# laoreja/HPLFlowNet

Hardware: AMD Instinct MI355X
Metric: point-pairs/sec + EPE3D, N=8192 FlyingThings3D, 1/2/4/8 MI355X (higher is better)
Workload: dtype f32 (wide layers: fp32 operands as scaled fp16 pairs, 3 partial products, fp32 accumulate); 1 GPU; full HPLFlowNet inference (7 levels, 19.3M params, random init), FT3D-like synthetic pair, N=8192, bs=1 per GPU; num_points=8192, step_includes_lattice_build=True, forward_streams=3, lattices_under_construction=3, exact_fallback_launches=0, lattice_launches_per_pair=34

## Files before the change

hplflownet_amd/csrc/gconv3.hip:

```cpp
#include "common.h"
#include "gconv_common.h"

#include <stdlib.h>
#include <string>
#include <type_traits>

using namespace hpl;
using namespace hpl_gc;

typedef __bf16 bf16x8 __attribute__((ext_vector_type(8)));
typedef __bf16 bf16x2 __attribute__((ext_vector_type(2)));
typedef _Float16 f16x8 __attribute__((ext_vector_type(8)));
typedef _Float16 f16x2 __attribute__((ext_vector_type(2)));
typedef float float2_t __attribute__((ext_vector_type(2)));
typedef unsigned u32x4 __attribute__((ext_vector_type(4)));
typedef unsigned u32x2 __attribute__((ext_vector_type(2)));


namespace {

__device__ __forceinline__ void split2(float x0, float x1, unsigned &h, unsigned &m, unsigned &l) {
    const float2_t v = {x0, x1};
    h = __builtin_bit_cast(unsigned, __builtin_convertvector(v, bf16x2));
    const float r0 = x0 - __builtin_bit_cast(float, h << 16), r1 = x1 - __builtin_bit_cast(float, h & 0xffff0000u);
    const float2_t rv = {r0, r1};
    m = __builtin_bit_cast(unsigned, __builtin_convertvector(rv, bf16x2));
    const float s0 = r0 - __builtin_bit_cast(float, m << 16), s1 = r1 - __builtin_bit_cast(float, m & 0xffff0000u);
    const float2_t sv = {s0, s1};
    l = __builtin_bit_cast(unsigned, __builtin_convertvector(sv, bf16x2));
}

__device__ __forceinline__ void split2h(float x0, float x1, float s, unsigned &h, unsigned &l) {
    const float2_t v = {x0 * s, x1 * s};
    const f16x2 hh = __builtin_convertvector(v, f16x2);
    h = __builtin_bit_cast(unsigned, hh);
    const float2_t hf = __builtin_convertvector(hh, float2_t);
    const float2_t r = {v.x - hf.x, v.y - hf.y};
    l = __builtin_bit_cast(unsigned, __builtin_convertvector(r, f16x2));
}

__device__ __forceinline__ void split2h_resid(float x0, float x1, float s, unsigned &h, unsigned &l) {
    const float2_t v = {x0 * s, x1 * s};
    const f16x2 hh = __builtin_convertvector(v, f16x2);
    const float2_t hf = __builtin_convertvector(hh, float2_t);
    const float2_t r = {v.x - hf.x, v.y - hf.y};
    const f16x2 ll = __builtin_convertvector(r, f16x2);
    const float2_t lf = __builtin_convertvector(ll, float2_t);
    constexpr float K = (float)(1 << RESID_SHIFT);
    const float2_t r2 = {(r.x - lf.x) * K, (r.y - lf.y) * K};
    const f16x2 h2 = __builtin_convertvector(r2, f16x2);
    h = __builtin_bit_cast(unsigned, h2);
    const float2_t h2f = __builtin_convertvector(h2, float2_t);
    const float2_t q = {r2.x - h2f.x, r2.y - h2f.y};
    l = __builtin_bit_cast(unsigned, __builtin_convertvector(q, f16x2));
}

constexpr int BM3 = 128;

template <int WGN, int F_LDS, int NB, int PL, bool GUARD = false>
__device__ __forceinline__ void gconv3_body(const GParams &p, const unsigned block) {
    static_assert(PL == 2 || PL == 3, "operand planes: 2 (fp16 pairs) or 3 (bf16 triples)");
    static_assert(!GUARD || PL == 2, "the range guard belongs to the fp16-pair form");
    bool tripped = false;
    if constexpr (PL == 2) tripped = guard_tripped(p.a_amax, p.a_guard);
    if constexpr (GUARD) { if (!tripped) return; }
    constexpr int BM = BM3, BN = 64 * WGN, NT = 128 * WGN;
    constexpr int ROWS_PP = NT / 4;
    constexpr int A_PASSES = 2 * BM / ROWS_PP;
    constexpr int HALF_PASSES = A_PASSES / 2;
    constexpr int A_STAGE = PL * 2 * BM * 16;
    constexpr int B_STAGE = PL * 2 * BN * 16;
    constexpr int NA = 3;
    static_assert(NB == 3 || NB == 4, "weight ring of 3 or 4 stages");
    constexpr int ASETS = NB - 1;
    constexpr int B_BASE = NA * A_STAGE;
    constexpr int B_CHUNKS_PER_WAVE = PL;
    constexpr int KLIST = 1024;
    constexpr bool PP = WGN == 4;
    static_assert(A_PASSES == 2 || A_PASSES == 4, "two halves of a slice per thread");
    __shared__ __attribute__((aligned(16))) unsigned char smem[NA * A_STAGE + NB * B_STAGE + ((F_LDS + 1) * BM + BM + 8) * 4 + KLIST * 2];
    int *Is = reinterpret_cast<int *>(smem + NA * A_STAGE + NB * B_STAGE);
    int *Vs = Is + (F_LDS + 1) * BM;
    int *tapmask_s = Vs + BM;
    unsigned short *Ks = reinterpret_cast<unsigned short *>(tapmask_s + 8);

    int tile_m, tile_n;
    tile_coords(p, tile_m, tile_n, block);
    if (tile_m < 0) return;
    const int64_t m0 = (int64_t)tile_m * BM;
    const int n0 = tile_n * BN;
    const int t = threadIdx.x, lane = t & 63;
    const int wave = __builtin_amdgcn_readfirstlane(t >> 6);
    const int wm = wave / WGN, wn = wave % WGN;
    const int li = lane & 31, hi = lane >> 5;

    const bool probe = p.clock_probe && (block & 63) == 0 && t == 0;
    long long probe_c = 0, probe_w = 0;
    if (probe) { probe_c = (long long)__builtin_readcyclecounter(); probe_w = (long long)__builtin_amdgcn_s_memrealtime(); }

    if (p.tile_idx && p.tile_bm == BM) {
        const int32_t *ti = p.tile_idx + (int64_t)tile_m * p.F * BM;
        if (t < 8) tapmask_s[t] = p.tile_mask[(int64_t)tile_m * 8 + t];
        for (int r = t; r < BM; r += NT) {
            const int64_t m = m0 + r;
            Vs[r] = (m < p.M) ? (p.row_perm ? p.row_perm[m] : (int)m) : -1;
        }
        for (int i = t; i < (F_LDS + 1) * BM; i += NT) {
            const int row = (i < p.F * BM) ? ti[i] : -1;
            Is[i] = row >= 0 ? row * (int)(p.lda * 4) : (int)0x80000000;
        }
    } else {
        if (t < 8) tapmask_s[t] = 0;
        for (int r = t; r < BM; r += NT) {
            const int64_t m = m0 + r;
            Vs[r] = (m < p.M) ? (p.row_perm ? p.row_perm[m] : (int)m) : -1;
        }
        __syncthreads();
        int mybits = 0;
        for (int i = t; i < F_LDS * BM; i += NT) {
            const int f = i / BM, r = i - f * BM;
            const int v = Vs[r];
            int row = -1;
            if (v >= 0 && f < p.F) row = p.nbr ? p.nbr[(int64_t)f * p.nbr_stride + v] : (int)((int64_t)f * p.reg_stride + v);
            Is[i] = row >= 0 ? row * (int)(p.lda * 4) : (int)0x80000000;
            mybits |= (row >= 0) ? (1 << f) : 0;
        }
        for (int i = F_LDS * BM + t; i < (F_LDS + 1) * BM; i += NT) Is[i] = (int)0x80000000;
        if (mybits) {
            atomicOr(tapmask_s, mybits);
            atomicOr(tapmask_s + 2 + ((t % BM) >> 5), mybits);
        }
    }
    __syncthreads();
    const int tapmask = __builtin_amdgcn_readfirstlane(tapmask_s[0]);
    const bool blockskip = p.C >= BK;
    int bmask[2];
#pragma unroll
    for (int i = 0; i < 2; ++i) bmask[i] = __builtin_amdgcn_readfirstlane(tapmask_s[2 + wm * 2 + i]);
    const int nk = (p.K + BK - 1) / BK;
    if (wave == 0) {
        int count = 0;
        for (int base = 0; base < nk; base += 64) {
            const int kt = base + lane;
            bool need = false;
            int f_lo = 0;
            if (kt < nk) {
                f_lo = (kt * BK) / p.C;
                const int f_hi = min((kt * BK + BK - 1) / p.C, p.F - 1);
                int bits = 0;
                for (int f = f_lo; f <= f_hi; ++f) bits |= 1 << f;
                need = (tapmask & bits) != 0;
            }
            const unsigned long long bal = __ballot(need);
            if (need) {
                int e = kt;
                e |= (f_lo << 10) | ((blockskip && (kt * BK + BK - 1) / p.C > f_lo && f_lo + 1 < p.F) ? (1 << 14) : 0);
                Ks[count + __popcll(bal & ((1ull << lane) - 1ull))] = (unsigned short)e;
            }
            count += __popcll(bal);
        }
        if (lane == 0) tapmask_s[1] = count;
    }
    __syncthreads();
    int nsl = __builtin_amdgcn_readfirstlane(tapmask_s[1]);
    int split = 0;
    if (p.splits > 1) {
        const int ngrid = p.row_perm && p.col_share > 0 ? p.tiles_n * p.col_share * p.col_rows : p.tiles_m * p.tiles_n;
        split = (int)block / ngrid;
        const int k_lo = (int)((int64_t)nk * split / p.splits), k_hi = (int)((int64_t)nk * (split + 1) / p.splits);
        auto below = [&](int kt) {
            int a = 0, b = nsl;
            while (a < b) {
                const int mid = (a + b) >> 1;
                if ((int)(Ks[mid] & 1023) < kt) a = mid + 1; else b = mid;
            }
            return a;
        };
        const int lo = below(k_lo), hi_e = below(k_hi);
        __syncthreads();
        if (lo > 0) {
            unsigned short mine[KLIST / (128 * WGN) + 1];
            int cnt = 0;
            for (int i = t; i < hi_e - lo; i += NT) mine[cnt++] = Ks[lo + i];
            __syncthreads();
            cnt = 0;
            for (int i = t; i < hi_e - lo; i += NT) Ks[i] = mine[cnt++];
        }
        __syncthreads();
        nsl = hi_e - lo;
    }

    constexpr unsigned OOB = 0x80000000u;
    const int32x4_t rsrc_a = make_rsrc(p.A, (int)p.a_bytes);
    const int k4 = t & 3, arow0 = t >> 2;
    const unsigned w3_bytes = (unsigned)(p.w_bytes / 2);
    __amdgpu_buffer_rsrc_t rsrc_b[PL];
#pragma unroll
    for (int pl = 0; pl < PL; ++pl)
        rsrc_b[pl] = __builtin_amdgcn_make_buffer_rsrc(
            const_cast<unsigned char *>(reinterpret_cast<const unsigned char *>(p.Wt3) + (int64_t)pl * p.w3_plane_stride),
            (short)0, (int)w3_bytes, 0x00020000);
    const unsigned ldw16 = (unsigned)p.ldw * 16u;

    float4_t ra[ASETS][A_PASSES];
    int a_rows[A_PASSES], a_c[A_PASSES];
    auto load_a_rows = [&](int e) {
        const int f0 = (e >> 10) & 15;
        const int c0 = (e & 1023) * BK - f0 * p.C;
#pragma unroll
        for (int i = 0; i < A_PASSES; ++i) {
            int c = c0 + ((i & 1) * 4 + k4) * 4, f = f0;
            const bool wrap = c >= p.C;
            c = wrap ? c - p.C : c;
            f += wrap ? 1 : 0;
            a_rows[i] = Is[f * BM + arow0 + (i >> 1) * ROWS_PP];
            a_c[i] = c;
        }
    };
    auto load_a_issue = [&](auto set_tag) {
        constexpr int SET = decltype(set_tag)::value;
        const int32x4_t rs = rsrc_a;
#pragma unroll
        for (int i = 0; i < A_PASSES; ++i) {
            float4_t &dst = ra[SET][i];
            const unsigned o = (unsigned)a_rows[i] + (unsigned)a_c[i] * 4u;
            asm volatile("buffer_load_dwordx4 %0, %1, %2, 0 offen" : "=v"(dst) : "v"(o), "s"(rs) : "memory");
        }
    };
    auto load_a = [&](auto set_tag, int e) {
        load_a_rows(e);
        load_a_issue(set_tag);
    };
    auto pin = [&](auto set_tag) {
        constexpr int SET = decltype(set_tag)::value;
#pragma unroll
        for (int i = 0; i < A_PASSES; ++i) {
            float4_t &x = ra[SET][i];
            asm volatile("" : "+v"(x));
        }
    };
    auto a_slot = [](int row, int kb) { return row ^ ((((row >> 5) & 3) << 1) ^ (kb << 2)); };
    const int kb_w = (t >> 1) & 1;
    float s_a = 1.f, s_out = 1.f, s_out2 = 1.f;
    if constexpr (PL == 2) {
        s_a = split_scale(p.a_amax[0]);
        s_out = split_unscale(s_a);
        if constexpr (GUARD) s_out *= 1.0f / (float)(1 << RESID_SHIFT);
        s_out2 = split_unscale(split_scale(p.w_amax[0]));
    }
    auto store_a = [&](auto set_tag, int h, int st, int j) {
        constexpr int SET = decltype(set_tag)::value;
        const float4_t v = h ? ra[SET][2 * j + 1] : ra[SET][2 * j];
        const int row = arow0 + j * ROWS_PP;
        unsigned char *base = smem + st * A_STAGE + (kb_w * BM + a_slot(row, kb_w)) * 16 + (t & 1) * 8;
        if constexpr (PL == 2) {
            unsigned h0, l0, h1, l1;
            if constexpr (GUARD) {
                split2h_resid(v.x, v.y, s_a, h0, l0);
                split2h_resid(v.z, v.w, s_a, h1, l1);
            } else {
                split2h(v.x, v.y, s_a, h0, l0);
                split2h(v.z, v.w, s_a, h1, l1);
            }
            *reinterpret_cast<u32x2 *>(base) = u32x2{h0, h1};
            *reinterpret_cast<u32x2 *>(base + 2 * BM * 16) = u32x2{l0, l1};
        } else {
            unsigned h0, m0_, l0, h1, m1, l1;
            split2(v.x, v.y, h0, m0_, l0);
            split2(v.z, v.w, h1, m1, l1);
            *reinterpret_cast<u32x2 *>(base) = u32x2{h0, h1};
            *reinterpret_cast<u32x2 *>(base + 2 * BM * 16) = u32x2{m0_, m1};
            *reinterpret_cast<u32x2 *>(base + 4 * BM * 16) = u32x2{l0, l1};
        }
    };
    const unsigned b_colofs = ((unsigned)(n0 + wn * 64 + lane) < (unsigned)p.ldw) ? (unsigned)(n0 + wn * 64 + lane) * 16u : OOB;
    auto load_b = [&](int kt, int h, int st) {
        const unsigned kbg = (unsigned)(kt * (BK / 8) + h * 2 + wm);
        const unsigned off = kbg * ldw16 + b_colofs;
#pragma unroll
        for (int pl = 0; pl < PL; ++pl)
            __builtin_amdgcn_raw_ptr_buffer_load_lds(
                rsrc_b[pl],
                (__attribute__((address_space(3))) void *)(smem + B_BASE + st * B_STAGE + ((pl * 2 + wm) * BN + wn * 64) * 16),
                16, (int)off, 0, 0, 0);
    };

    floatx16 acc[2][2];
#pragma unroll
    for (int i = 0; i < 2; ++i)
#pragma unroll
        for (int j = 0; j < 2; ++j)
#pragma unroll
            for (int r = 0; r < 16; ++r) acc[i][j][r] = 0.f;

    unsigned a_rofs[2];
#pragma unroll
    for (int i = 0; i < 2; ++i) {
        const int row = wm * 64 + i * 32 + li;
        a_rofs[i] = (unsigned)((hi * BM + (row ^ ((((row >> 5) & 3) << 1) ^ (hi << 2)))) * 16);
    }
    const unsigned b_rofs = (unsigned)(B_BASE + (hi * BN + wn * 64 + li) * 16);

    using S0 = std::integral_constant<int, 0>;
    using S1 = std::integral_constant<int, 1>;
    using T = std::true_type;
    using Fl = std::false_type;
    auto wait_vm_lgkm0 = [](auto n_tag) {
        constexpr int N = decltype(n_tag)::value;
        __builtin_amdgcn_s_waitcnt((N & 0xF) | ((N >> 4) << 14) | (0x7 << 4) | (0x0 << 8));
    };

    using S2 = std::integral_constant<int, 2>;
    if (nsl > 0) {
        int ks_cb = 0;
        int ks_reg = (int)Ks[min(lane, KLIST - 1)];
        auto ks_at = [&](int x) { return __builtin_amdgcn_readlane(ks_reg, x - ks_cb); };
        auto ks_advance = [&](int sl) {
            if (sl - ks_cb >= 32) { ks_cb += 32; ks_reg = (int)Ks[min(ks_cb + lane, KLIST - 1)]; }
        };
        auto kt_at = [&](int sl) { return ks_at(sl) & 1023; };
#pragma unroll
        for (int g = 0; g < NB - 1; ++g)
            if (g / 2 < nsl) load_b(kt_at(g / 2), g & 1, g);
        load_a(S0{}, ks_at(0));
        wait_vm_lgkm0(S0{});
        pin(S0{});
#pragma unroll
        for (int j = 0; j < HALF_PASSES; ++j) { store_a(S0{}, 0, 0, j); store_a(S0{}, 1, 1, j); }
        if (nsl > 1) load_a(S1{}, ks_at(1));
        if constexpr (ASETS == 3) { if (nsl > 2) load_a(S2{}, ks_at(2)); }
        wait_vm_lgkm0(S0{});
        asm volatile("s_barrier" ::: "memory");

        if (PP && wm == 1) asm volatile("s_barrier" ::: "memory");

        int sta = 0, stb = 0;
        auto halfstep = [&](int e_cur, int h, auto b_tag, int kt_b, int hb_b, auto w_tag, auto setw_tag, auto l_tag, auto setl_tag,
                            int kt_l, auto inflight_tag) {
            constexpr bool B = decltype(b_tag)::value, W = decltype(w_tag)::value, L = decltype(l_tag)::value;
            const int sta2 = sta >= 1 ? sta - 1 : 2;
            const int stb2 = stb >= 1 ? stb - 1 : NB - 1;
            const unsigned char *sa = smem + sta * A_STAGE;
            const unsigned char *sb = smem + stb * B_STAGE;
            bool need[2];
            {
                const int f_lo = (e_cur >> 10) & 15, two = (e_cur >> 14) & 1;
#pragma unroll
                for (int i = 0; i < 2; ++i)
                    need[i] = !blockskip || (((bmask[i] >> f_lo) | (two ? (bmask[i] >> (f_lo + 1)) : 0)) & 1);
            }
            u32x4 af[PL][2], bf[PL][2];
            constexpr int NQ = PL == 3 ? 6 : 3;
            constexpr int PA[6] = {0, 0, 1, 0, PL == 3 ? 2 : 0, 1};
            constexpr int PB[6] = {0, 1, 0, PL == 3 ? 2 : 0, 0, 1};
            auto mfma = [&](const u32x4 &a, const u32x4 &b, floatx16 &c) {
                if constexpr (PL == 3)
                    c = __builtin_amdgcn_mfma_f32_32x32x16_bf16(__builtin_bit_cast(bf16x8, b), __builtin_bit_cast(bf16x8, a), c, 0, 0, 0);
                else
                    c = __builtin_amdgcn_mfma_f32_32x32x16_f16(__builtin_bit_cast(f16x8, b), __builtin_bit_cast(f16x8, a), c, 0, 0, 0);
            };
            if constexpr (PP) {
#pragma unroll
                for (int pl = 0; pl < PL; ++pl)
#pragma unroll
                    for (int i = 0; i < 2; ++i) {
                        af[pl][i] = *reinterpret_cast<const u32x4 *>(sa + a_rofs[i] + pl * 2 * BM * 16);
                        bf[pl][i] = *reinterpret_cast<const u32x4 *>(sb + b_rofs + pl * 2 * BN * 16 + i * 32 * 16);
                    }
                wait_vm_lgkm0(inflight_tag);
                __builtin_amdgcn_sched_barrier(0);
                asm volatile("s_barrier" ::: "memory");
                __builtin_amdgcn_sched_barrier(0);
                auto others = [&]() {
                    if constexpr (B) load_b(kt_b, hb_b, stb2);
                    if constexpr (L) { load_a_issue(setl_tag); load_a_rows(kt_l); }
                    if constexpr (W) {
                        if (h == 0) pin(setw_tag);
#pragma unroll
                        for (int j = 0; j < HALF_PASSES; ++j) store_a(setw_tag, h, sta2, j);
                    }
                };
                if (need[0] || need[1]) {
#pragma unroll
                    for (int q = 0; q < NQ; ++q)
#pragma unroll
                        for (int i = 0; i < 2; ++i)
#pragma unroll
                            for (int j = 0; j < 2; ++j) mfma(af[PA[q]][i], bf[PB[q]][j], acc[i][j]);
                    others();
#pragma unroll
                    for (int k = 0; k < 4 * NQ; ++k) {
                        __builtin_amdgcn_sched_group_barrier(0x008, 1, 0);
                        __builtin_amdgcn_sched_group_barrier(0x006, 4, 0);
                        if (k % 3 == 0) __builtin_amdgcn_sched_group_barrier(0x020, 1, 0);
                        if (k % 4 == 1) __builtin_amdgcn_sched_group_barrier(0x100, 1, 0);
                        if (k % 4 == 3) __builtin_amdgcn_sched_group_barrier(0x200, 1, 0);
                    }
                } else {
                    others();
                }
                __builtin_amdgcn_sched_barrier(0);
                asm volatile("s_barrier" ::: "memory");
                __builtin_amdgcn_sched_barrier(0);
                sta = sta == 2 ? 0 : sta + 1;
                stb = stb == NB - 1 ? 0 : stb + 1;
                return;
            }
            if (need[0] || need[1]) {
#pragma unroll
                for (int pl = 0; pl < PL; ++pl)
#pragma unroll
                    for (int i = 0; i < 2; ++i) {
                        af[pl][i] = *reinterpret_cast<const u32x4 *>(sa + a_rofs[i] + pl * 2 * BM * 16);
                        bf[pl][i] = *reinterpret_cast<const u32x4 *>(sb + b_rofs + pl * 2 * BN * 16 + i * 32 * 16);
                    }
            }
            if constexpr (B) load_b(kt_b, hb_b, stb2);
            if constexpr (L) load_a_rows(kt_l);
            if constexpr (W) { if (h == 0) pin(setw_tag); }
            auto rest = [&]() {
                if constexpr (L) load_a_issue(setl_tag);
                if constexpr (W) {
#pragma unroll
                    for (int j = 0; j < HALF_PASSES; ++j) store_a(setw_tag, h, sta2, j);
                }
            };
            if (need[0] || need[1]) {
#pragma unroll
                for (int q = 0; q < NQ; ++q)
#pragma unroll
                    for (int i = 0; i < 2; ++i)
#pragma unroll
                        for (int j = 0; j < 2; ++j) mfma(af[PA[q]][i], bf[PB[q]][j], acc[i][j]);
                rest();
#pragma unroll
                for (int k = 0; k < 4 * NQ; ++k) {
                    __builtin_amdgcn_sched_group_barrier(0x008, 1, 0);
                    __builtin_amdgcn_sched_group_barrier(0x006, 4, 0);
                    if (k % 4 == 0) __builtin_amdgcn_sched_group_barrier(0x020, 1, 0);
                    if (k % 4 == 3) __builtin_amdgcn_sched_group_barrier(0x200, 1, 0);
                }
            } else {
                rest();
            }
            wait_vm_lgkm0(inflight_tag);
            asm volatile("s_barrier" ::: "memory");
            sta = sta == 2 ? 0 : sta + 1;
            stb = stb == NB - 1 ? 0 : stb + 1;
        };
        constexpr int NLB = B_CHUNKS_PER_WAVE, NLA = A_PASSES;
        auto slice_steady = [&](int sl, auto u_tag) {
            constexpr int U = decltype(u_tag)::value;
            using SW = std::integral_constant<int, (U + 1) % ASETS>;
            using SL = std::integral_constant<int, U % ASETS>;
            ks_advance(sl);
            const int e = ks_at(sl);
            const int k1 = kt_at(sl + 1), kl = ks_at(sl + ASETS);
            if constexpr (PP) {
                halfstep(e, 0, T{}, k1, 1, T{}, SW{}, T{}, SL{}, ks_at(sl + ASETS + 1), std::integral_constant<int, NLB>{});
                halfstep(e, 1, T{}, kt_at(sl + 2), 0, T{}, SW{}, Fl{}, SL{}, 0, std::integral_constant<int, NLB + NLA>{});
            } else
            if constexpr (NB == 3) {
                halfstep(e, 0, T{}, k1, 0, T{}, SW{}, T{}, SL{}, kl, std::integral_constant<int, NLB + NLA>{});
                halfstep(e, 1, T{}, k1, 1, T{}, SW{}, Fl{}, SL{}, 0, std::integral_constant<int, NLB>{});
            } else {
                halfstep(e, 0, T{}, k1, 1, T{}, SW{}, T{}, SL{}, kl, std::integral_constant<int, 2 * NLB + NLA>{});
                halfstep(e, 1, T{}, kt_at(sl + 2), 0, T{}, SW{}, Fl{}, SL{}, 0, std::integral_constant<int, 2 * NLB + NLA>{});
            }
        };
        auto slice_tail = [&](int sl, auto u_tag) {
            constexpr int U = decltype(u_tag)::value;
            using SW = std::integral_constant<int, (U + 1) % ASETS>;
            using SL = std::integral_constant<int, U % ASETS>;
            using Z = std::integral_constant<int, 0>;
            ks_advance(sl);
            const int e = ks_at(sl);
            const bool w = sl + 1 < nsl, l = sl + ASETS < nsl;
            const int kl = l ? ks_at(sl + ASETS + (PP ? 1 : 0)) : 0;
            {
                const int gb = 2 * sl + NB - 1;
                const bool b = gb / 2 < nsl;
                const int kb = b ? kt_at(gb / 2) : 0;
                if (b && w && l) halfstep(e, 0, T{}, kb, gb & 1, T{}, SW{}, T{}, SL{}, kl, Z{});
                else if (b && w) halfstep(e, 0, T{}, kb, gb & 1, T{}, SW{}, Fl{}, SL{}, 0, Z{});
                else if (w) halfstep(e, 0, Fl{}, 0, 0, T{}, SW{}, Fl{}, SL{}, 0, Z{});
                else if (b) halfstep(e, 0, T{}, kb, gb & 1, Fl{}, SW{}, Fl{}, SL{}, 0, Z{});
                else halfstep(e, 0, Fl{}, 0, 0, Fl{}, SW{}, Fl{}, SL{}, 0, Z{});
            }
            {
                const int gb = 2 * sl + 1 + NB - 1;
                const bool b = gb / 2 < nsl;
                const int kb = b ? kt_at(gb / 2) : 0;
                if (b && w) halfstep(e, 1, T{}, kb, gb & 1, T{}, SW{}, Fl{}, SL{}, 0, Z{});
                else if (w) halfstep(e, 1, Fl{}, 0, 0, T{}, SW{}, Fl{}, SL{}, 0, Z{});
                else if (b) halfstep(e, 1, T{}, kb, gb & 1, Fl{}, SW{}, Fl{}, SL{}, 0, Z{});
                else halfstep(e, 1, Fl{}, 0, 0, Fl{}, SW{}, Fl{}, SL{}, 0, Z{});
            }
        };
        if constexpr (PP) load_a_rows(ks_at(ASETS));
        int sl = 0;
        for (; sl + 2 * ASETS < nsl; sl += ASETS) {
            slice_steady(sl, S0{});
            slice_steady(sl + 1, S1{});
            if constexpr (ASETS == 3) slice_steady(sl + 2, S2{});
        }
        for (; sl < nsl; sl += ASETS) {
            slice_tail(sl, S0{});
            if (sl + 1 < nsl) slice_tail(sl + 1, S1{});
            if constexpr (ASETS == 3) { if (sl + 2 < nsl) slice_tail(sl + 2, S2{}); }
        }
        if (PP && wm == 0) asm volatile("s_barrier" ::: "memory");
    }
    if constexpr (PL == 2) {
#pragma unroll
        for (int i = 0; i < 2; ++i)
#pragma unroll
            for (int j = 0; j < 2; ++j)
#pragma unroll
                for (int r = 0; r < 16; ++r) acc[i][j][r] = acc[i][j][r] * s_out * s_out2;
    }
    if constexpr (GUARD) {
        if (p.guard_trips && t == 0 && tile_m == 0 && tile_n == 0 && split == 0) atomicAdd(p.guard_trips, 1);
    }
    const bool defer = !GUARD && tripped;

    typedef int int32x4v __attribute__((ext_vector_type(4)));
    const bool fast_epi = p.epi_fast != 0;
    if (fast_epi) {
        const __amdgpu_buffer_rsrc_t rs_y = __builtin_amdgcn_make_buffer_rsrc(
            p.splits > 1 ? (void *)(p.partial + (int64_t)split * p.M * p.N) : (void *)p.Y, (short)0, 0x7fffffff, 0x00020000);
        const __amdgpu_buffer_rsrc_t rs_r = __builtin_amdgcn_make_buffer_rsrc(
            p.res ? (void *)const_cast<float *>(p.res) : (void *)p.Y, (short)0, p.res ? 0x7fffffff : 0, 0x00020000);
        const __amdgpu_buffer_rsrc_t rs_y2 = __builtin_amdgcn_make_buffer_rsrc(
            p.Y2 ? (void *)p.Y2 : (void *)p.Y, (short)0, (p.Y2 && p.splits <= 1) ? 0x7fffffff : 0, 0x00020000);
        const unsigned ldy_b = (unsigned)(p.splits > 1 ? p.N : p.ldy) * 4u, ldr_b = (unsigned)p.ldres * 4u, ldy2_b = (unsigned)p.ldy2 * 4u;
        const bool plain = p.splits <= 1;
        unsigned ymax = 0;
        unsigned gmin = 0xffffffffu;
        const bool want_guard = p.y_guard && p.y_amax && plain && !defer;
        const bool res_wrap = p.res && p.res_mod < p.M;
        const float res_inv = res_wrap ? 1.0f / (float)p.res_mod : 0.f;
        const bool has_res = p.res != nullptr && plain;
        const bool has_y2 = p.Y2 != nullptr && plain && !defer;
        int mrow[2];
        unsigned yrow[2], rrow[2], y2row[2];
#pragma unroll
        for (int i = 0; i < 2; ++i) {
            const int m = Vs[wm * 64 + i * 32 + li];
            mrow[i] = m;
            int rr = m;
            if (res_wrap) {
                const int q = (int)((float)rr * res_inv);
                rr -= (int)__umul24((unsigned)q, (unsigned)p.res_mod);
                rr = rr < 0 ? rr + (int)p.res_mod : (rr >= (int)p.res_mod ? rr - (int)p.res_mod : rr);
            }
            yrow[i] = __umul24((unsigned)m, ldy_b);
            rrow[i] = __umul24((unsigned)rr, ldr_b);
            y2row[i] = __umul24((unsigned)m, ldy2_b);
        }
        auto at = [&](int m, unsigned row_b, int n) { return (m >= 0 && n < p.N) ? row_b + (unsigned)n * 4u : OOB; };
        auto col_of = [&](int j, int q) { return n0 + wn * 64 + j * 32 + 8 * q + 4 * hi; };
        u32x4 rv[2][2][4];
        if (has_res) {
#pragma unroll
            for (int i = 0; i < 2; ++i)
#pragma unroll
                for (int j = 0; j < 2; ++j)
#pragma unroll
                    for (int q = 0; q < 4; ++q)
                        rv[i][j][q] = __builtin_amdgcn_raw_buffer_load_b128(rs_r, (int)at(mrow[i], rrow[i], col_of(j, q)), 0, 0);
        }
#pragma unroll
        for (int i = 0; i < 2; ++i) {
            unsigned rowmax = 0;
#pragma unroll
            for (int j = 0; j < 2; ++j)
#pragma unroll
                for (int q = 0; q < 4; ++q) {
                    const int n = col_of(j, q);
                    float4_t bs = {0.f, 0.f, 0.f, 0.f};
                    if (p.bias && plain && n < p.N) bs = *reinterpret_cast<const float4_t *>(p.bias + n);
                    float v[4] = {acc[i][j][4 * q + 0], acc[i][j][4 * q + 1], acc[i][j][4 * q + 2], acc[i][j][4 * q + 3]};
                    const float bb[4] = {bs.x, bs.y, bs.z, bs.w};
                    const unsigned rr4[4] = {rv[i][j][q].x, rv[i][j][q].y, rv[i][j][q].z, rv[i][j][q].w};
                    u32x4 o;
                    unsigned ob[4];
                    const bool live = mrow[i] >= 0 && n < p.N;
#pragma unroll
                    for (int c = 0; c < 4; ++c) {
                        float x = v[c];
                        if (plain) {
                            x = x + bb[c];
                            if (has_res) x += __builtin_bit_cast(float, rr4[c]);
                            if (p.act == HPL_ACT_LEAKY && !defer) x = x > 0.f ? x : p.slope * x;
                        }
                        ob[c] = __builtin_bit_cast(unsigned, x);
                        const unsigned av = live ? (ob[c] & 0x7fffffffu) : 0u;
                        ymax = max(ymax, av);
                        rowmax = max(rowmax, av);
                    }
                    o.x = ob[0]; o.y = ob[1]; o.z = ob[2]; o.w = ob[3];
                    __builtin_amdgcn_raw_buffer_store_b128(o, rs_y, (int)at(mrow[i], yrow[i], n), 0, 0);
                    if (has_y2) __builtin_amdgcn_raw_buffer_store_b128(o, rs_y2, (int)at(mrow[i] < (int)p.rows2 ? mrow[i] : -1, y2row[i], n), 0, 0);
                }
            if (want_guard) {
                rowmax = max(rowmax, (unsigned)__shfl_xor((int)rowmax, 32));
                gmin = rowmax ? min(gmin, rowmax) : gmin;
            }
        }
        if (p.y_amax && plain && !defer) {
#pragma unroll
            for (int o = 32; o > 0; o >>= 1) ymax = max(ymax, (unsigned)__shfl_xor((int)ymax, o));
            unsigned inv = 0u;
            if (want_guard) {
                inv = gmin == 0xffffffffu ? 0u : ~gmin;
#pragma unroll
                for (int o = 16; o > 0; o >>= 1) inv = max(inv, (unsigned)__shfl_xor((int)inv, o));
            }
            __syncthreads();
            unsigned *red = reinterpret_cast<unsigned *>(smem);
            if (lane == 0) { red[2 * wave] = ymax; red[2 * wave + 1] = inv; }
            __syncthreads();
            if (t == 0) {
#pragma unroll
                for (int w = 1; w < NT / 64; ++w) { ymax = max(ymax, red[2 * w]); inv = max(inv, red[2 * w + 1]); }
                amax_publish(reinterpret_cast<unsigned *>(p.y_amax), ymax);
                if (want_guard) amax_publish(p.y_guard, inv);
            }
        }
    } else
#pragma unroll
    for (int i = 0; i < 2; ++i)
#pragma unroll
        for (int j = 0; j < 2; ++j) {
            const int64_t m = Vs[wm * 64 + i * 32 + li];
            if (m < 0) continue;
            const int res_mod = (int)p.res_mod;
#pragma unroll
            for (int r = 0; r < 16; ++r) {
                const int n = n0 + wn * 64 + j * 32 + (r & 3) + 8 * (r >> 2) + 4 * hi;
                if (n >= p.N) continue;
                const float bsv = p.bias ? p.bias[n] : 0.f;
                if (p.splits > 1) {
                    p.partial[((int64_t)split * p.M + m) * p.N + n] = acc[i][j][r];
                    continue;
                }
                float v = acc[i][j][r] + bsv;
                if (p.res) v += p.res[(int64_t)((int)m < res_mod ? (int)m : (int)m % res_mod) * p.ldres + n];
                if (p.act == HPL_ACT_LEAKY && !defer) v = v > 0.f ? v : p.slope * v;
                p.Y[m * p.ldy + n] = v;
                if (p.Y2 && m < p.rows2 && !defer) p.Y2[m * p.ldy2 + n] = v;
            }
        }
    if (probe) {
        atomicAdd(reinterpret_cast<unsigned long long *>(p.clock_probe),
                  (unsigned long long)((long long)__builtin_readcyclecounter() - probe_c));
        atomicAdd(reinterpret_cast<unsigned long long *>(p.clock_probe) + 1,
                  (unsigned long long)((long long)__builtin_amdgcn_s_memrealtime() - probe_w));
    }
}

template <int WGN, int F_LDS, int PL, int NB = 3, bool GUARD = false>
__global__ void __launch_bounds__(128 * WGN, 2) k_gconv3(const GParams p) {
    gconv3_body<WGN, F_LDS, NB, PL, GUARD>(p, blockIdx.x);
}

template <int F_LDS, int NB, int PL, bool GUARD = false>
__global__ void __launch_bounds__(512, 2) k_gconv3w(const GParams p) {
    gconv3_body<4, F_LDS, NB, PL, GUARD>(p, blockIdx.x);
}

__global__ void __launch_bounds__(256) k_weight_split3(const float *__restrict__ Wt, int64_t k_rows, int64_t ldw,
                                                        unsigned char *__restrict__ dst, int64_t plane_stride) {
    const int64_t total = (k_rows / 8) * ldw;
    int64_t i = (int64_t)blockIdx.x * blockDim.x + threadIdx.x;
    const int64_t stride = (int64_t)gridDim.x * blockDim.x;
    for (; i < total; i += stride) {
        const int64_t kb = i / ldw, n = i - kb * ldw;
        float x[8];
#pragma unroll
        for (int j = 0; j < 8; ++j) x[j] = Wt[(kb * 8 + j) * ldw + n];
        u32x4 h, m, l;
        unsigned a, b, c;
        split2(x[0], x[1], a, b, c); h.x = a; m.x = b; l.x = c;
        split2(x[2], x[3], a, b, c); h.y = a; m.y = b; l.y = c;
        split2(x[4], x[5], a, b, c); h.z = a; m.z = b; l.z = c;
        split2(x[6], x[7], a, b, c); h.w = a; m.w = b; l.w = c;
        *reinterpret_cast<u32x4 *>(dst + i * 16) = h;
        *reinterpret_cast<u32x4 *>(dst + plane_stride + i * 16) = m;
        *reinterpret_cast<u32x4 *>(dst + 2 * plane_stride + i * 16) = l;
    }
}

__device__ __forceinline__ void amax_reduce(unsigned v, unsigned *slot) {
#pragma unroll
    for (int o = 32; o > 0; o >>= 1) v = max(v, (unsigned)__shfl_xor((int)v, o));
    __shared__ unsigned part[4];
    if ((threadIdx.x & 63) == 0) part[threadIdx.x >> 6] = v;
    __syncthreads();
    if (threadIdx.x == 0) {
        v = max(max(part[0], part[1]), max(part[2], part[3]));
        amax_publish(slot, v);
    }
}

template <typename V>
__global__ void __launch_bounds__(256) k_amax(const float *__restrict__ X, int64_t ld, int64_t rows, int colsv, int tpr_log, unsigned *__restrict__ slot) {
    constexpr int VW = sizeof(V) / 4;
    const int tpr = 1 << tpr_log, c0 = threadIdx.x & (tpr - 1), rpb = 256 >> tpr_log;
    unsigned v = 0;
    auto fold = [&](const V &x) {
        const unsigned *e = reinterpret_cast<const unsigned *>(&x);
#pragma unroll
        for (int u = 0; u < VW; ++u) v = max(v, e[u] & 0x7fffffffu);
    };
    const int64_t rstep = (int64_t)gridDim.x * rpb;
    int64_t r = (int64_t)blockIdx.x * rpb + (threadIdx.x >> tpr_log);
    for (; r + 3 * rstep < rows; r += 4 * rstep) {
        const float *p0 = X + r * ld, *p1 = p0 + rstep * ld, *p2 = p1 + rstep * ld, *p3 = p2 + rstep * ld;
        for (int c = c0; c < colsv; c += tpr) {
            const V a = *reinterpret_cast<const V *>(p0 + (int64_t)c * VW), b = *reinterpret_cast<const V *>(p1 + (int64_t)c * VW);
            const V d = *reinterpret_cast<const V *>(p2 + (int64_t)c * VW), f = *reinterpret_cast<const V *>(p3 + (int64_t)c * VW);
            fold(a); fold(b); fold(d); fold(f);
        }
    }
    for (; r < rows; r += rstep) {
        const float *p0 = X + r * ld;
        for (int c = c0; c < colsv; c += tpr) fold(*reinterpret_cast<const V *>(p0 + (int64_t)c * VW));
    }
    amax_reduce(v, slot);
}

template <typename V>
__global__ void __launch_bounds__(256) k_amax_rows(const float *__restrict__ X, int64_t ld, int64_t rows, int colsv, int tpr_log,
                                                   unsigned *__restrict__ slot, unsigned *__restrict__ guard) {
    constexpr int VW = sizeof(V) / 4;
    const int tpr = 1 << tpr_log, c0 = threadIdx.x & (tpr - 1), rpb = 256 >> tpr_log;
    unsigned v = 0, ginv = 0;
    auto fold = [&](unsigned &m, const V &x) {
        const unsigned *e = reinterpret_cast<const unsigned *>(&x);
#pragma unroll
        for (int u = 0; u < VW; ++u) m = max(m, e[u] & 0x7fffffffu);
    };
    auto row_done = [&](unsigned m) {
        for (int o = tpr >> 1; o > 0; o >>= 1) m = max(m, (unsigned)__shfl_xor((int)m, o));
        v = max(v, m);
        ginv = m ? max(ginv, ~m) : ginv;
    };
    const int64_t rstep = (int64_t)gridDim.x * rpb;
    for (int64_t r = (int64_t)blockIdx.x * rpb + (threadIdx.x >> tpr_log); r < rows; r += 4 * rstep) {
        const int64_t r1 = r + rstep < rows ? r + rstep : r, r2 = r + 2 * rstep < rows ? r + 2 * rstep : r, r3 = r + 3 * rstep < rows ? r + 3 * rstep : r;
        const float *p0 = X + r * ld, *p1 = X + r1 * ld, *p2 = X + r2 * ld, *p3 = X + r3 * ld;
        unsigned m0 = 0, m1 = 0, m2 = 0, m3 = 0;
        for (int c = c0; c < colsv; c += tpr) {
            const V a = *reinterpret_cast<const V *>(p0 + (int64_t)c * VW), b = *reinterpret_cast<const V *>(p1 + (int64_t)c * VW);
            const V d = *reinterpret_cast<const V *>(p2 + (int64_t)c * VW), f = *reinterpret_cast<const V *>(p3 + (int64_t)c * VW);
            fold(m0, a); fold(m1, b); fold(m2, d); fold(m3, f);
        }
        row_done(m0); row_done(m1); row_done(m2); row_done(m3);
    }
#pragma unroll
    for (int o = 32; o > 0; o >>= 1) ginv = max(ginv, (unsigned)__shfl_xor((int)ginv, o));
    __shared__ unsigned gpart[4];
    if ((threadIdx.x & 63) == 0) gpart[threadIdx.x >> 6] = ginv;
    amax_reduce(v, slot);
    if (threadIdx.x == 0) amax_publish(guard, max(max(gpart[0], gpart[1]), max(gpart[2], gpart[3])));
}

__global__ void k_amax_clear(const hpl_split3_job *__restrict__ jobs, int njobs) {
    for (int j = threadIdx.x; j < njobs; j += blockDim.x)
        if (jobs[j].planes == 2 && jobs[j].amax) *jobs[j].amax = 0.f;
}

__global__ void __launch_bounds__(256) k_amax_batch(const hpl_split3_job *__restrict__ jobs) {
    const hpl_split3_job jb = jobs[blockIdx.y];
    unsigned v = 0;
    if (jb.planes == 2) {
        const int64_t total4 = jb.k_rows * jb.ldw / 4;
        const uint4 *X = reinterpret_cast<const uint4 *>(jb.Wt);
        for (int64_t i = (int64_t)blockIdx.x * 256 + threadIdx.x; i < total4; i += (int64_t)gridDim.x * 256) {
            const uint4 x = X[i];
            v = max(max(v, x.x & 0x7fffffffu), max(max(x.y & 0x7fffffffu, x.z & 0x7fffffffu), x.w & 0x7fffffffu));
        }
    }
    amax_reduce(v, reinterpret_cast<unsigned *>(jb.amax ? jb.amax : const_cast<float *>(jb.Wt)));
}

__device__ __forceinline__ void split2h_store(const float *x, float sc, unsigned char *dst, int64_t plane_stride, int64_t i) {
    u32x4 h, l;
    unsigned a, b;
    split2h(x[0], x[1], sc, a, b); h.x = a; l.x = b;
    split2h(x[2], x[3], sc, a, b); h.y = a; l.y = b;
    split2h(x[4], x[5], sc, a, b); h.z = a; l.z = b;
    split2h(x[6], x[7], sc, a, b); h.w = a; l.w = b;
    *reinterpret_cast<u32x4 *>(dst + i * 16) = h;
    *reinterpret_cast<u32x4 *>(dst + plane_stride + i * 16) = l;
}

__global__ void __launch_bounds__(256) k_weight_split2h(const float *__restrict__ Wt, int64_t k_rows, int64_t ldw,
                                                         unsigned char *__restrict__ dst, int64_t plane_stride,
                                                         const float *__restrict__ amax) {
    const float sc = split_scale(amax[0]);
    const int64_t total = (k_rows / 8) * ldw;
    for (int64_t i = (int64_t)blockIdx.x * 256 + threadIdx.x; i < total; i += (int64_t)gridDim.x * 256) {
        const int64_t kb = i / ldw, n = i - kb * ldw;
        float x[8];
#pragma unroll
        for (int j = 0; j < 8; ++j) x[j] = Wt[(kb * 8 + j) * ldw + n];
        split2h_store(x, sc, dst, plane_stride, i);
    }
}

}

__global__ void __launch_bounds__(256) k_weight_split3_batch(const hpl_split3_job *__restrict__ jobs) {
    const hpl_split3_job jb = jobs[blockIdx.y];
    const float *Wt = jb.Wt;
    unsigned char *dst = reinterpret_cast<unsigned char *>(jb.dst);
    const int64_t ldw = jb.ldw, total = (jb.k_rows / 8) * ldw;
    const float sc = jb.planes == 2 ? split_scale(jb.amax[0]) : 1.f;
    for (int64_t i = (int64_t)blockIdx.x * 256 + threadIdx.x; i < total; i += (int64_t)gridDim.x * 256) {
        const int64_t kb = i / ldw, n = i - kb * ldw;
        float x[8];
#pragma unroll
        for (int j = 0; j < 8; ++j) x[j] = Wt[(kb * 8 + j) * ldw + n];
        if (jb.planes == 2) { split2h_store(x, sc, dst, jb.plane_stride, i); continue; }
        u32x4 h, m, l;
        unsigned a, b, c;
        split2(x[0], x[1], a, b, c); h.x = a; m.x = b; l.x = c;
        split2(x[2], x[3], a, b, c); h.y = a; m.y = b; l.y = c;
        split2(x[4], x[5], a, b, c); h.z = a; m.z = b; l.z = c;
        split2(x[6], x[7], a, b, c); h.w = a; m.w = b; l.w = c;
        *reinterpret_cast<u32x4 *>(dst + i * 16) = h;
        *reinterpret_cast<u32x4 *>(dst + jb.plane_stride + i * 16) = m;
        *reinterpret_cast<u32x4 *>(dst + 2 * jb.plane_stride + i * 16) = l;
    }
}

extern "C" int hpl_weight_split3_batch(const hpl_split3_job *jobs, int njobs, int64_t max_elems, int any_pairs, hplStream stream) {
    HPL_REQUIRE(jobs && njobs > 0 && njobs <= 65535 && max_elems > 0, "hpl_weight_split3_batch: bad arguments");
    if (any_pairs) {
        k_amax_clear<<<1, 256, 0, to_stream(stream)>>>(jobs, njobs);
        dim3 ga((unsigned)imin(cdiv(max_elems / 4, 256), 256), (unsigned)njobs);
        k_amax_batch<<<ga, 256, 0, to_stream(stream)>>>(jobs);
    }
    dim3 grid((unsigned)imin(cdiv(max_elems / 8, 256), 2048), (unsigned)njobs);
    k_weight_split3_batch<<<grid, 256, 0, to_stream(stream)>>>(jobs);
    HPL_CHECK_LAUNCH("hpl_weight_split3_batch");
    return HPL_OK;
}

int hpl_gc::amax_launch(const float *X, int64_t ld, int64_t rows, int cols, float *slot, hipStream_t s, unsigned *guard) {
    if (rows <= 0) return HPL_OK;
    const bool vec = cols % 4 == 0 && ld % 4 == 0 && aligned16(X);
    int cv = vec ? cols / 4 : cols;
    int64_t nrows = rows;
    if (guard) {
        int tl = 0;
        while ((1 << tl) < cv && tl < 6) ++tl;
        const int rpb = 256 >> tl;
        const int grid = (int)imax(1, imin(cdiv(nrows, (int64_t)rpb * 4), 1024));
        if (vec) k_amax_rows<float4><<<grid, 256, 0, s>>>(X, ld, nrows, cv, tl, reinterpret_cast<unsigned *>(slot), guard);
        else k_amax_rows<float><<<grid, 256, 0, s>>>(X, ld, nrows, cv, tl, reinterpret_cast<unsigned *>(slot), guard);
        HPL_CHECK_LAUNCH("hpl_amax_rows");
        return HPL_OK;
    }
    if (ld == cols && (int64_t)rows * cv >= 256) {
        const int64_t total = rows * cv;
        int w = 256;
        while (total % w) w >>= 1;
        if (w >= 64) { cv = w; nrows = total / w; ld = (int64_t)w * (vec ? 4 : 1); }
    }
    int tpr_log = 0;
    while ((1 << tpr_log) < cv && tpr_log < 8) ++tpr_log;
    const int rpb = 256 >> tpr_log;
    const int grid = (int)imax(1, imin(cdiv(nrows, (int64_t)rpb * 4), 1024));
    if (vec) k_amax<float4><<<grid, 256, 0, s>>>(X, ld, nrows, cv, tpr_log, reinterpret_cast<unsigned *>(slot));
    else k_amax<float><<<grid, 256, 0, s>>>(X, ld, nrows, cv, tpr_log, reinterpret_cast<unsigned *>(slot));
    HPL_CHECK_LAUNCH("hpl_amax");
    return HPL_OK;
}

extern "C" int hpl_amax(const float *X, int64_t ld, int64_t rows, int32_t cols, float *slot, hplStream stream) {
    HPL_REQUIRE(X && slot && rows >= 0 && cols > 0 && ld >= cols, "hpl_amax: bad arguments (rows=%lld cols=%d ld=%lld)", (long long)rows, cols, (long long)ld);
    hipStream_t s = to_stream(stream);
    if (hipMemsetAsync(slot, 0, 4, s) != hipSuccess) { set_error("hpl_amax: hipMemsetAsync failed"); return HPL_EHIP; }
    return amax_launch(X, ld, rows, cols, slot, s);
}

extern "C" int hpl_amax_rows(const float *X, int64_t ld, int64_t rows, int32_t cols, float *slot, uint32_t *guard, hplStream stream) {
    HPL_REQUIRE(X && slot && guard && rows >= 0 && cols > 0 && ld >= cols, "hpl_amax_rows: bad arguments (rows=%lld cols=%d ld=%lld)", (long long)rows, cols, (long long)ld);
    hipStream_t s = to_stream(stream);
    if (hipMemsetAsync(slot, 0, 4, s) != hipSuccess || hipMemsetAsync(guard, 0, 4, s) != hipSuccess) { set_error("hpl_amax_rows: hipMemsetAsync failed"); return HPL_EHIP; }
    return amax_launch(X, ld, rows, cols, slot, s, guard);
}

extern "C" int hpl_weight_split2h(const float *Wt, int64_t k_rows, int64_t ldw, void *dst, int64_t plane_stride, float *amax,
                                  hplStream stream) {
    HPL_REQUIRE(Wt && dst && amax && k_rows > 0 && k_rows % 8 == 0 && ldw > 0 && plane_stride >= k_rows * ldw * 2 &&
                    plane_stride % 16 == 0 && aligned16(dst),
                "hpl_weight_split2h: bad arguments (k_rows=%lld ldw=%lld)", (long long)k_rows, (long long)ldw);
    const int rc = hpl_amax(Wt, ldw, k_rows, (int32_t)ldw, amax, stream);
    if (rc) return rc;
    const int grid = (int)imin(cdiv(k_rows / 8 * ldw, 256), 16384);
    k_weight_split2h<<<grid, 256, 0, to_stream(stream)>>>(Wt, k_rows, ldw, reinterpret_cast<unsigned char *>(dst), plane_stride, amax);
    HPL_CHECK_LAUNCH("hpl_weight_split2h");
    return HPL_OK;
}

extern "C" int hpl_weight_split3(const float *Wt, int64_t k_rows, int64_t ldw, void *dst, int64_t plane_stride,
                                 hplStream stream) {
    HPL_REQUIRE(Wt && dst && k_rows > 0 && k_rows % 8 == 0 && ldw > 0 && plane_stride >= k_rows * ldw * 2 &&
                    plane_stride % 16 == 0 && aligned16(dst),
                "hpl_weight_split3: bad arguments (k_rows=%lld ldw=%lld)", (long long)k_rows, (long long)ldw);
    const int grid = (int)imin(cdiv(k_rows / 8 * ldw, 256), 16384);
    k_weight_split3<<<grid, 256, 0, to_stream(stream)>>>(Wt, k_rows, ldw, reinterpret_cast<unsigned char *>(dst), plane_stride);
    HPL_CHECK_LAUNCH("hpl_weight_split3");
    return HPL_OK;
}

bool hpl_gc::split3_enabled() { return split_planes() != 0; }

int hpl_gc::split_planes() {
    static const int planes = [] {
        const char *m = getenv("HPL_MATH");
        if (m && std::string(m) == "f32") return 0;
        if (m && std::string(m) == "bf16x3") return 3;
        return 2;
    }();
    return planes;
}

bool hpl_gc::launch_split3(GParams &p, hipStream_t s) {
    if (!split3_enabled() || p.scat || p.C < 32 || p.K > 32768) return false;
    if (p.F > 15 || (p.w_bytes / (p.ldw * 4)) % 8 != 0) return false;
    constexpr int min_rows = 8192;
    constexpr int min_rows_stencil = 16384;
    constexpr int fill_tiles = 128;
    constexpr int floor_rows = 1024;
    if (p.N < 256 || p.M < floor_rows) return false;
    const int64_t tiles256 = cdiv(p.M, BM3) * cdiv(p.N, 256);
    const bool fills = tiles256 >= fill_tiles;
    if (p.F == 1 && p.M < min_rows && !fills) return false;
    int splitk = 1;
    if (p.F > 1 && p.M < min_rows_stencil && !fills) {
        constexpr int mid_split = 1;
        constexpr int mid_min_rows = 1024;
        if (p.M < mid_min_rows) return false;
        const int64_t tiles = tiles256;
        const int nk_all = (p.K + BK - 1) / BK;
        splitk = (int)imin(imin(8, 256 / imax(1, tiles)), nk_all / 16);
        const int sets = (p.planes == 2 && p.a_guard) ? 2 : 1;
        if (!mid_split || !p.ws || p.scat || splitk < 2 || (int64_t)sets * splitk * p.M * p.N * 4 > p.ws_bytes || p.N % 256 > 0) return false;
    }
    p.tiles_m = (int)cdiv(p.M, BM3);
    constexpr int wide = 256;
    constexpr int pct = 108;
    const bool bn256 = splitk > 1 || (wide == 256 && cdiv(p.N, 256) * 256 * 100 <= cdiv(p.N, 128) * 128 * pct);
    const int BN = bn256 ? 256 : 128;
    p.tiles_n = (int)cdiv(p.N, BN);
    if (p.tile_bm != BM3) p.tile_idx = nullptr;
    p.splits = 1; p.partial = nullptr;
    int grid = p.tiles_m * p.tiles_n;
    p.col_share = 0; p.col_rows = 0;
    if (splitk > 1) {
        p.splits = splitk;
        p.partial = p.ws;
    }
    if (p.row_perm) {
        int g = 8, b = p.tiles_n % 8;
        while (b) { const int tt = g % b; g = b; b = tt; }
        p.col_share = 8 / g;
        p.col_rows = p.col_share == 1 ? p.tiles_m : (int)cdiv(p.tiles_m, COL_CHUNK * p.col_share) * COL_CHUNK;
        grid = p.tiles_n * p.col_share * p.col_rows;
        constexpr int xcd_row_major = 1;
        if (xcd_row_major && p.splits <= 1 && p.tiles_n > 1 && p.tiles_n <= 8) {
            p.col_share = -1;
            p.col_rows = (int)cdiv(p.tiles_m, 8);
            grid = 8 * p.col_rows * p.tiles_n;
        }
    }
    grid *= p.splits;
    {
        const int64_t lim = (int64_t)0x7fffffff;
        const int64_t rows_y = p.M;
        p.epi_fast = (rows_y < (1 << 24) && rows_y * (p.splits > 1 ? p.N : p.ldy) * 4 < lim && p.ldy * 4 < (1 << 24) &&
                      (!p.res || (p.res_mod > 0 && p.res_mod < (1 << 24) && imin(p.res_mod, rows_y) * p.ldres * 4 < lim && p.ldres * 4 < (1 << 24))) &&
                      (!p.Y2 || (p.rows2 * p.ldy2 * 4 < lim && p.ldy2 * 4 < (1 << 24))) &&
                      p.N % 4 == 0 && (p.splits > 1 ? aligned16(p.partial) : (p.ldy % 4 == 0 && aligned16(p.Y))) && (!p.bias || aligned16(p.bias)) &&
                      (!p.res || (p.ldres % 4 == 0 && aligned16(p.res))) && (!p.Y2 || (p.ldy2 % 4 == 0 && aligned16(p.Y2)))) ? 1 : 0;
        static const int epi = getenv("HPL_SPLIT3_EPILOGUE") ? atoi(getenv("HPL_SPLIT3_EPILOGUE")) : 1;
        if (!epi) p.epi_fast = 0;
    }
    p.y_amax_done = (p.y_amax && p.epi_fast && p.splits <= 1) ? 1 : 0;
    if (p.planes == 2) {
        if (bn256) {
            if (p.F == 1) k_gconv3w<1, 4, 2><<<grid, 512, 0, s>>>(p);
            else if (p.F <= 8) k_gconv3w<8, 4, 2><<<grid, 512, 0, s>>>(p);
            else k_gconv3w<15, 4, 2><<<grid, 512, 0, s>>>(p);
        } else {
            if (p.F == 1) k_gconv3<2, 1, 2><<<grid, 256, 0, s>>>(p);
            else if (p.F <= 8) k_gconv3<2, 8, 2><<<grid, 256, 0, s>>>(p);
            else k_gconv3<2, 15, 2><<<grid, 256, 0, s>>>(p);
        }
        if (p.a_guard) {
            GParams q = p;
            const int ggrid = grid;
            if (p.splits > 1) { q.partial = p.partial + (int64_t)p.splits * p.M * p.N; p.guard_partials = 1; }
            else { q.res = p.Y; q.ldres = p.ldy; q.res_mod = p.M; q.bias = nullptr; }
            if (bn256) {
                if (p.F == 1) k_gconv3w<1, 4, 2, true><<<ggrid, 512, 0, s>>>(q);
                else if (p.F <= 8) k_gconv3w<8, 4, 2, true><<<ggrid, 512, 0, s>>>(q);
                else k_gconv3w<15, 4, 2, true><<<ggrid, 512, 0, s>>>(q);
            } else {
                if (p.F == 1) k_gconv3<2, 1, 2, 3, true><<<ggrid, 256, 0, s>>>(q);
                else if (p.F <= 8) k_gconv3<2, 8, 2, 3, true><<<ggrid, 256, 0, s>>>(q);
                else k_gconv3<2, 15, 2, 3, true><<<ggrid, 256, 0, s>>>(q);
            }
        }
    } else if (bn256) {
        if (p.F == 1) k_gconv3w<1, 4, 3><<<grid, 512, 0, s>>>(p);
        else if (p.F <= 8) k_gconv3w<8, 4, 3><<<grid, 512, 0, s>>>(p);
        else k_gconv3w<15, 4, 3><<<grid, 512, 0, s>>>(p);
    } else {
        if (p.F == 1) k_gconv3<2, 1, 3><<<grid, 256, 0, s>>>(p);
        else if (p.F <= 8) k_gconv3<2, 8, 3><<<grid, 256, 0, s>>>(p);
        else k_gconv3<2, 15, 3><<<grid, 256, 0, s>>>(p);
    }
    return true;
}
```

Measured before the change: 446.7 point-pairs/s.

## Replace full-tile guard residual GEMM with a lean single-wave residual kernel

The residual-guard pass, which runs only when the activation range guard trips, no longer relaunches the full LDS-pipelined gconv3 tile kernel. It now uses a dedicated 64-thread kernel that loads activations and weights directly into MFMA 32x32x16 fp16 ops with a grid-stride loop. When the guard does not trip, the old path still launched a full grid of heavy 512/256-thread blocks that each returned early; the new kernel exits just as early but with small blocks and a capped grid, so it costs less launch and occupancy. The main kernel also loses its GUARD template branches. The tripped path is now an unpipelined kernel without LDS reuse and may be slower when the guard actually fires.

Measured after the change: 460.9 point-pairs/s (median of 6 runs). 1.03x the previous value.

```diff
diff --git a/hplflownet_amd/csrc/gconv3.hip b/hplflownet_amd/csrc/gconv3.hip
--- a/hplflownet_amd/csrc/gconv3.hip
+++ b/hplflownet_amd/csrc/gconv3.hip
@@ -57,13 +57,11 @@
 
 constexpr int BM3 = 128;
 
-template <int WGN, int F_LDS, int NB, int PL, bool GUARD = false>
+template <int WGN, int F_LDS, int NB, int PL>
 __device__ __forceinline__ void gconv3_body(const GParams &p, const unsigned block) {
     static_assert(PL == 2 || PL == 3, "operand planes: 2 (fp16 pairs) or 3 (bf16 triples)");
-    static_assert(!GUARD || PL == 2, "the range guard belongs to the fp16-pair form");
     bool tripped = false;
     if constexpr (PL == 2) tripped = guard_tripped(p.a_amax, p.a_guard);
-    if constexpr (GUARD) { if (!tripped) return; }
     constexpr int BM = BM3, BN = 64 * WGN, NT = 128 * WGN;
     constexpr int ROWS_PP = NT / 4;
     constexpr int A_PASSES = 2 * BM / ROWS_PP;
@@ -245,7 +243,6 @@
     if constexpr (PL == 2) {
         s_a = split_scale(p.a_amax[0]);
         s_out = split_unscale(s_a);
-        if constexpr (GUARD) s_out *= 1.0f / (float)(1 << RESID_SHIFT);
         s_out2 = split_unscale(split_scale(p.w_amax[0]));
     }
     auto store_a = [&](auto set_tag, int h, int st, int j) {
@@ -255,13 +252,8 @@
         unsigned char *base = smem + st * A_STAGE + (kb_w * BM + a_slot(row, kb_w)) * 16 + (t & 1) * 8;
         if constexpr (PL == 2) {
             unsigned h0, l0, h1, l1;
-            if constexpr (GUARD) {
-                split2h_resid(v.x, v.y, s_a, h0, l0);
-                split2h_resid(v.z, v.w, s_a, h1, l1);
-            } else {
-                split2h(v.x, v.y, s_a, h0, l0);
-                split2h(v.z, v.w, s_a, h1, l1);
-            }
+            split2h(v.x, v.y, s_a, h0, l0);
+            split2h(v.z, v.w, s_a, h1, l1);
             *reinterpret_cast<u32x2 *>(base) = u32x2{h0, h1};
             *reinterpret_cast<u32x2 *>(base + 2 * BM * 16) = u32x2{l0, l1};
         } else {
@@ -519,10 +511,7 @@
 #pragma unroll
                 for (int r = 0; r < 16; ++r) acc[i][j][r] = acc[i][j][r] * s_out * s_out2;
     }
-    if constexpr (GUARD) {
-        if (p.guard_trips && t == 0 && tile_m == 0 && tile_n == 0 && split == 0) atomicAdd(p.guard_trips, 1);
-    }
-    const bool defer = !GUARD && tripped;
+    const bool defer = tripped;
 
     typedef int int32x4v __attribute__((ext_vector_type(4)));
     const bool fast_epi = p.epi_fast != 0;
@@ -660,14 +649,128 @@
     }
 }
 
-template <int WGN, int F_LDS, int PL, int NB = 3, bool GUARD = false>
+template <int WGN, int F_LDS, int PL, int NB = 3>
 __global__ void __launch_bounds__(128 * WGN, 2) k_gconv3(const GParams p) {
-    gconv3_body<WGN, F_LDS, NB, PL, GUARD>(p, blockIdx.x);
-}
-
-template <int F_LDS, int NB, int PL, bool GUARD = false>
+    gconv3_body<WGN, F_LDS, NB, PL>(p, blockIdx.x);
+}
+
+template <int F_LDS, int NB, int PL>
 __global__ void __launch_bounds__(512, 2) k_gconv3w(const GParams p) {
-    gconv3_body<4, F_LDS, NB, PL, GUARD>(p, blockIdx.x);
+    gconv3_body<4, F_LDS, NB, PL>(p, blockIdx.x);
+}
+
+__global__ void __launch_bounds__(64) __attribute__((amdgpu_waves_per_eu(8, 8))) k_gconv3_resid(const GParams p) {
+    if (!guard_tripped(p.a_amax, p.a_guard)) return;
+    const int lane = threadIdx.x, li = lane & 31, hi = lane >> 5;
+    const int split = blockIdx.y;
+    if (p.guard_trips && blockIdx.x == 0 && split == 0 && lane == 0) atomicAdd(p.guard_trips, 1);
+    constexpr unsigned OOB = 0x80000000u;
+    const int32x4_t rs_a = make_rsrc(p.A, (int)p.a_bytes);
+    const int32x4_t rs_wh = make_rsrc(p.Wt3, (int)(p.w_bytes / 2));
+    const int32x4_t rs_wl = make_rsrc(reinterpret_cast<const unsigned char *>(p.Wt3) + p.w3_plane_stride, (int)(p.w_bytes / 2));
+    const float s_a = split_scale(p.a_amax[0]);
+    const int nk = (p.K + BK - 1) / BK;
+    const int k_lo = (int)((int64_t)nk * split / p.splits) * BK, k_hi = (int)((int64_t)nk * (split + 1) / p.splits) * BK;
+    const int f_lo = k_lo / p.C, c_lo = k_lo - f_lo * p.C;
+    const unsigned units_n = (unsigned)(p.N + 63) / 64u, units = (unsigned)((p.M + 31) / 32) * units_n;
+    const bool split_k = p.splits > 1;
+    auto row_of = [&](int f, int v) -> unsigned {
+        if (v < 0 || f >= p.F) return OOB;
+        const int row = p.nbr ? p.nbr[(int64_t)f * p.nbr_stride + v] : (int)((int64_t)f * p.reg_stride + v);
+        return row >= 0 ? (unsigned)row * ((unsigned)p.lda * 4u) : OOB;
+    };
+    for (unsigned u = blockIdx.x; u < units; u += gridDim.x) {
+        const unsigned um = u / units_n, un = u - um * units_n;
+        const unsigned m = um * 32u + (unsigned)li;
+        const int v = (int64_t)m < p.M ? (p.row_perm ? p.row_perm[m] : (int)m) : -1;
+        unsigned ymax = 0;
+#pragma unroll 1
+        for (int j = 0; j < 2; ++j) {
+            const int n0 = (int)un * 64 + j * 32;
+            if (n0 >= p.N) break;
+            int f0 = f_lo, c0 = c_lo + 8 * hi;
+            if (c0 >= p.C) { c0 -= p.C; ++f0; }
+            unsigned r0 = row_of(f0, v);
+            floatx16 acc;
+#pragma unroll
+            for (int r = 0; r < 16; ++r) acc[r] = 0.f;
+#pragma unroll 1
+            for (int k = k_lo; k < k_hi; k += 16) {
+                const bool ends = c0 + 4 >= p.C;
+                const unsigned r1 = ends ? row_of(f0 + 1, v) : r0 + (unsigned)(c0 + 4) * 4u;
+                const float4_t x0 = buffer_load_f32x4(rs_a, (int)(r0 + (unsigned)c0 * 4u), 0, 0);
+                const float4_t x1 = buffer_load_f32x4(rs_a, (int)r1, 0, 0);
+                unsigned h0, l0, h1, l1, h2, l2, h3, l3;
+                split2h_resid(x0.x, x0.y, s_a, h0, l0);
+                split2h_resid(x0.z, x0.w, s_a, h1, l1);
+                split2h_resid(x1.x, x1.y, s_a, h2, l2);
+                split2h_resid(x1.z, x1.w, s_a, h3, l3);
+                const u32x4 ah = {h0, h1, h2, h3}, al = {l0, l1, l2, l3};
+                __builtin_amdgcn_sched_barrier(0);
+                const unsigned wc = (unsigned)(n0 + li);
+                const unsigned w_off = wc < (unsigned)p.ldw ? ((unsigned)(k / 8 + hi) * (unsigned)p.ldw + wc) * 16u : OOB;
+                const float4_t wh = buffer_load_f32x4(rs_wh, (int)w_off, 0, 0);
+                const float4_t wl = buffer_load_f32x4(rs_wl, (int)w_off, 0, 0);
+                const f16x8 a_h = __builtin_bit_cast(f16x8, ah), a_l = __builtin_bit_cast(f16x8, al);
+                const f16x8 w_h = __builtin_bit_cast(f16x8, wh), w_l = __builtin_bit_cast(f16x8, wl);
+                acc = __builtin_amdgcn_mfma_f32_32x32x16_f16(w_h, a_h, acc, 0, 0, 0);
+                acc = __builtin_amdgcn_mfma_f32_32x32x16_f16(w_l, a_h, acc, 0, 0, 0);
+                acc = __builtin_amdgcn_mfma_f32_32x32x16_f16(w_h, a_l, acc, 0, 0, 0);
+                c0 += 16;
+                if (c0 >= p.C) { c0 -= p.C; ++f0; r0 = row_of(f0, v); }
+            }
+            if (v < 0) continue;
+            int ve = v;
+            asm volatile("" : "+v"(ve));
+            const float s_out = split_unscale(s_a) * (1.0f / (float)(1 << RESID_SHIFT)), s_out2 = split_unscale(split_scale(p.w_amax[0]));
+            float *yrow = split_k ? p.partial + ((int64_t)split * p.M + ve) * p.N : p.Y + (int64_t)ve * p.ldy;
+            float *y2row = (!split_k && p.Y2 && ve < p.rows2) ? p.Y2 + (int64_t)ve * p.ldy2 : nullptr;
+#pragma unroll
+            for (int q = 0; q < 4; ++q) {
+                const int n = n0 + 8 * q + 4 * hi;
+                if (n >= p.N) continue;
+                float4_t x = {acc[4 * q] * s_out * s_out2, acc[4 * q + 1] * s_out * s_out2, acc[4 * q + 2] * s_out * s_out2,
+                              acc[4 * q + 3] * s_out * s_out2};
+                auto finish = [&](float xs, float y) {
+                    xs += y;
+                    if (p.act == HPL_ACT_LEAKY) xs = xs > 0.f ? xs : p.slope * xs;
+                    ymax = max(ymax, __builtin_bit_cast(unsigned, xs) & 0x7fffffffu);
+                    return xs;
+                };
+                if (p.epi_fast) {
+                    if (!split_k) {
+                        const float4_t y = *reinterpret_cast<const float4_t *>(yrow + n);
+                        x.x = finish(x.x, y.x); x.y = finish(x.y, y.y); x.z = finish(x.z, y.z); x.w = finish(x.w, y.w);
+                    }
+                    *reinterpret_cast<float4_t *>(yrow + n) = x;
+                    if (y2row) *reinterpret_cast<float4_t *>(y2row + n) = x;
+                } else {
+#pragma unroll
+                    for (int c = 0; c < 4; ++c) {
+                        if (n + c >= p.N) break;
+                        float xs = x[c];
+                        if (!split_k) xs = finish(xs, yrow[n + c]);
+                        yrow[n + c] = xs;
+                        if (y2row) y2row[n + c] = xs;
+                    }
+                }
+            }
+        }
+        if (p.y_amax && p.y_amax_done && !split_k) {
+            const unsigned rowmax = max(ymax, (unsigned)__shfl_xor((int)ymax, 32));
+            unsigned inv = rowmax ? ~rowmax : 0u;
+            ymax = rowmax;
+#pragma unroll
+            for (int o = 16; o > 0; o >>= 1) {
+                ymax = max(ymax, (unsigned)__shfl_xor((int)ymax, o));
+                inv = max(inv, (unsigned)__shfl_xor((int)inv, o));
+            }
+            if (lane == 0) {
+                amax_publish(reinterpret_cast<unsigned *>(p.y_amax), ymax);
+                if (p.y_guard) amax_publish(p.y_guard, inv);
+            }
+        }
+    }
 }
 
 __global__ void __launch_bounds__(256) k_weight_split3(const float *__restrict__ Wt, int64_t k_rows, int64_t ldw,
@@ -934,6 +1037,7 @@
 bool hpl_gc::launch_split3(GParams &p, hipStream_t s) {
     if (!split3_enabled() || p.scat || p.C < 32 || p.K > 32768) return false;
     if (p.F > 15 || (p.w_bytes / (p.ldw * 4)) % 8 != 0) return false;
+    if (p.planes == 2 && p.a_guard && cdiv(p.M, 32) * cdiv(p.N, 64) > (int64_t)0x7fffffff) return false;
     constexpr int min_rows = 8192;
     constexpr int min_rows_stencil = 16384;
     constexpr int fill_tiles = 128;
@@ -1005,18 +1109,9 @@
         }
         if (p.a_guard) {
             GParams q = p;
-            const int ggrid = grid;
             if (p.splits > 1) { q.partial = p.partial + (int64_t)p.splits * p.M * p.N; p.guard_partials = 1; }
-            else { q.res = p.Y; q.ldres = p.ldy; q.res_mod = p.M; q.bias = nullptr; }
-            if (bn256) {
-                if (p.F == 1) k_gconv3w<1, 4, 2, true><<<ggrid, 512, 0, s>>>(q);
-                else if (p.F <= 8) k_gconv3w<8, 4, 2, true><<<ggrid, 512, 0, s>>>(q);
-                else k_gconv3w<15, 4, 2, true><<<ggrid, 512, 0, s>>>(q);
-            } else {
-                if (p.F == 1) k_gconv3<2, 1, 2, 3, true><<<ggrid, 256, 0, s>>>(q);
-                else if (p.F <= 8) k_gconv3<2, 8, 2, 3, true><<<ggrid, 256, 0, s>>>(q);
-                else k_gconv3<2, 15, 2, 3, true><<<ggrid, 256, 0, s>>>(q);
-            }
+            const int64_t units = cdiv(p.M, 32) * cdiv(p.N, 64);
+            k_gconv3_resid<<<dim3((unsigned)imin(units, imax(1, 4096 / p.splits)), (unsigned)p.splits), 64, 0, s>>>(q);
         }
     } else if (bn256) {
         if (p.F == 1) k_gconv3w<1, 4, 3><<<grid, 512, 0, s>>>(p);
```
